# Deci-AI/super-gradients

Measured on NVIDIA H100. Metric: images/sec YOLO-NAS-S 640 bf16 train, higher is better.
Workload: dtype bf16

## Files before the change

include/sgb200.h:

```cpp
#ifndef SGB200_H_
#define SGB200_H_

#include <stdint.h>

#ifdef __cplusplus
extern "C" {
#endif

#define SGB_OK 0
#define SGB_E_INVALID (-1)
#define SGB_E_UNSUPPORTED (-2)
#define SGB_E_CUDA (-3)
#define SGB_E_ARCH (-4)

#define SGB_ACT_NONE 0
#define SGB_ACT_RELU 1
#define SGB_ACT_SILU 2

typedef uint16_t sgb_bf16;

typedef struct SgbConvDesc {
  int32_t N, H, W, C;
  int32_t K, R, S;
  int32_t P, Q;
// ... 10 lines not shown
  const sgb_bf16* residual;
  double* stats;
  int32_t stats_repl;
  int32_t act;
  int32_t out_f32;
} SgbEpilogue;

const char* sgb_last_error(void);
int sgb_version(void);
int sgb_check_device(void);
int64_t sgb_sm100_launches(void);
int64_t sgb_conv_halo_launches(void);
void sgb_conv_force_im2col(int on);
int64_t sgb_conv_wgrad_halo_launches(void);
void sgb_conv_wgrad_force_im2col(int on);

int sgb_conv_fprop(const SgbConvDesc* d, const sgb_bf16* x, const sgb_bf16* w_krsc, void* y, const SgbEpilogue* ep,
                   void* stream);
int sgb_conv_dgrad(const SgbConvDesc* d, const sgb_bf16* dy, const sgb_bf16* w_crsk, sgb_bf16* dx, int accumulate,
                   void* stream);
int sgb_conv_wgrad(const SgbConvDesc* d, const sgb_bf16* x, const sgb_bf16* dy, float* dw_krsc, void* stream);
int sgb_weight_prepare(const float* w_oihw, int K, int C, int R, int S, int c_pad, sgb_bf16* w_krsc, sgb_bf16* w_crsk,
                       const float* scale, int add_identity, void* stream);
int sgb_wgrad_to_oihw(const float* dw_krsc, int K, int C, int R, int S, int c_pad, float* g_oihw, int accumulate,
                      void* stream);
typedef struct SgbWeightItem {
  const float* w;
  const float* scale;
  sgb_bf16* krsc;
  sgb_bf16* crsk;
// ... 402 lines not shown
```

super_gradients_b200/csrc/capi.cu:

```cuda
#include <cstdarg>
#include <cstdio>

#include "common.cuh"
#include "conv_sm100.h"
#include "sm100_host.h"

static thread_local char g_err[512] = "";

void sgb_set_error(const char* fmt, ...) {
  va_list ap;
  va_start(ap, fmt);
  vsnprintf(g_err, sizeof(g_err), fmt, ap);
  va_end(ap);
}

int sgb_cuda_check(cudaError_t e, const char* what) {
  if (e == cudaSuccess) return SGB_OK;
  sgb_set_error("%s: %s", what, cudaGetErrorString(e));
  return SGB_E_CUDA;
}

extern "C" const char* sgb_last_error(void) { return g_err; }
extern "C" int sgb_version(void) { return 100; }
extern "C" int sgb_check_device(void) {
// ... 1 lines not shown
  if (int rc = sgb_cuda_check(cudaGetDevice(&dev), "cudaGetDevice")) return rc;
  cudaDeviceProp prop;
  if (int rc = sgb_cuda_check(cudaGetDeviceProperties(&prop, dev), "cudaGetDeviceProperties")) return rc;
  if (prop.major != 9) {
    sgb_set_error("libsgb200 is built for sm_90a only; device is sm_%d%d", prop.major, prop.minor);
    return SGB_E_ARCH;
  }
  return SGB_OK;
}

extern "C" int64_t sgb_sm100_launches(void) { return (int64_t)sm100::launch_count(); }
extern "C" int64_t sgb_conv_halo_launches(void) { return (int64_t)sm100::halo_launch_count(); }
extern "C" void sgb_conv_force_im2col(int on) { sm100::force_im2col(on != 0); }
extern "C" int64_t sgb_conv_wgrad_halo_launches(void) { return (int64_t)sm100::wgrad_halo_launch_count(); }
extern "C" void sgb_conv_wgrad_force_im2col(int on) { sm100::wgrad_force_im2col(on != 0); }
```

super_gradients_b200/csrc/conv_mma.cu:

```cuda
#include "common.cuh"
#include "conv_sm100.h"

namespace {

constexpr int BM = 128;
constexpr int BK = 32;
constexpr int STAGES = 4;
constexpr int THREADS = 256;

struct GatherClass {
  int M;
  int Hc, Wc;
  int nr, ns;
  int Kg;
  int hb_add, wb_add;
  int r0, s0;
  int oh_add, ow_add;
};

struct IGemmParams {
  const bf16* A;
  const bf16* B;
  void* Y;
  GatherClass cls[4];
// ... 574 lines not shown
  SGB_REQUIRE(s == 1 || s == 2, "dgrad supports stride 1 or 2");
  const int Kp = ((d->K + 7) / 8) * 8;
  if (s == 1 && d->pad == d->R / 2 && d->K % 16 == 0) {
    sm100::Problem q{};
    q.a = dy + d->y_off; q.N = d->N; q.H = d->P; q.W = d->Q; q.C = d->K; q.a_pitch = d->y_pitch;
    q.b = w_crsk; q.b_rows = d->C; q.b_cols = d->R * d->S * Kp; q.b_cols_per_tap = Kp;
    q.R = d->R; q.S = d->S; q.stride = 1; q.pad = d->R - 1 - d->pad; q.P = d->H; q.Q = d->W; q.flip = 1;
    q.y = dx; q.y_pitch = d->x_pitch; q.y_off = d->x_off;
    q.residual = accumulate ? dx : nullptr;
    q.stats_repl = 1;
    q.centre_from = d->centre_from;
    if (sm100::supported(q)) return sm100::launch(q, (cudaStream_t)stream);
  }
  if (s == 2 && d->K % 16 == 0 && d->R == 3 && d->S == 3 && d->pad == 1 && d->C % 8 == 0 && d->H % 2 == 0 &&
      d->W % 2 == 0 && d->H == 2 * d->P && d->W == 2 * d->Q) {
    bool all_ok = true;
    for (int cls = 0; cls < 4 && all_ok; ++cls) {
      const int ph = cls >> 1, pw = cls & 1;
      sm100::Problem q{};
      q.a = dy + d->y_off; q.N = d->N; q.H = d->P; q.W = d->Q; q.C = d->K; q.a_pitch = d->y_pitch;
      q.b = w_crsk; q.b_rows = d->C; q.b_cols = d->R * d->S * Kp; q.b_cols_per_tap = Kp;
      q.R = d->R; q.S = d->S; q.stride = 1; q.pad = 0; q.P = d->P; q.Q = d->Q; q.flip = 0;
      q.y = dx; q.y_pitch = d->x_pitch; q.y_off = d->x_off;
      q.residual = accumulate ? dx : nullptr;
      q.stats_repl = 1;
      q.out_mode = 1; q.o_mul = 2; q.oh_add = ph; q.ow_add = pw; q.outH = d->H; q.outW = d->W;
      int nt = 0;
      for (int r = 0; r < d->R; ++r) {
        if (((ph + d->pad - r) & 1) != 0) continue;
        for (int sx = 0; sx < d->S; ++sx) {
// ... 135 lines not shown
```

super_gradients_b200/csrc/conv_sm100.cu:

```cuda
#include <cuda.h>

#include <cstdlib>
#include <cstring>

#include "common.cuh"
#include "conv_sm100.h"
#include "sm100_host.h"
#include "sm100_ptx.cuh"

namespace sm100 {

constexpr int BLOCK_M = 128;
constexpr int NUM_THREADS = 384;
constexpr int CONSUMER_THREADS = 256;
constexpr int MAX_STAGES = 8;

struct Params {
  int M;
  int N;
  int C;
  int KC;
  int n_tiles;
  int stages;
  int P, Q;
// ... 244 lines not shown
        row_ok[h] = m < p.M;
        orow[h] = out_row(p, row_ok[h] ? m : 0);
      }
      tile_epilogue<BN>(p, acc, orow, row_ok, nt, wg, wq, lane, s_part, s_stats);
    }
  }
  __syncthreads();
  flush_stats(p, s_stats);
}

constexpr int HALO_W = 10, HALO_H = 10, HALO_TILE = 8;
constexpr uint32_t HALO_CG_BYTES = 1664;
constexpr uint32_t HALO_CTRL_BYTES = CTRL_BAR_BYTES + 16;
constexpr int HALO_MAX_STAGES = 6;

template <int BN, bool SKIP>
__global__ void __launch_bounds__(NUM_THREADS, BN <= 48 ? 2 : 1)
conv3x3_halo_kernel(const __grid_constant__ CUtensorMap map_a, const __grid_constant__ CUtensorMap map_b, const Params p) {
  extern __shared__ __align__(1024) unsigned char smem_raw[];
  const uint32_t smem_base = (smem_u32(smem_raw) + 1023u) & ~1023u;
  const int ksteps = p.C / 16;
  constexpr uint32_t b_box = BN * 32;
  const uint32_t b_bytes = 9u * ksteps * b_box;
  const uint32_t a_stage = ((uint32_t)(p.C / 8) * HALO_CG_BYTES + 1023u) & ~1023u;
  const uint32_t sb = smem_base, sa0 = smem_base + ((b_bytes + 1023u) & ~1023u);
  const uint32_t ctrl = sa0 + p.stages * a_stage;
  auto full_bar = [&](int s) { return ctrl + 8u * s; };
  auto empty_bar = [&](int s) { return ctrl + 8u * (MAX_STAGES + s); };
  const uint32_t b_bar = ctrl + CTRL_BAR_BYTES;
  float* s_part = reinterpret_cast<float*>(smem_raw + (ctrl + HALO_CTRL_BYTES - smem_u32(smem_raw)));
  float* s_stats = s_part + 8 * 2 * BN;

  const int warp = threadIdx.x >> 5, lane = threadIdx.x & 31;
  const int m_tiles = p.M;
  const int nt = blockIdx.x % p.n_tiles;
  const int mt_step = gridDim.x / p.n_tiles;
  const int mt0 = blockIdx.x / p.n_tiles;
  const int off = SKIP ? off_centre_steps<BN>(p, nt, ksteps, 16) : ksteps;

// ... 4 lines not shown
    }
    mbar_init(b_bar, 1);
    asm volatile("fence.mbarrier_init.release.cluster;" ::: "memory");
    asm volatile("fence.proxy.async.shared::cta;" ::: "memory");
  }
  if (p.stats)
    for (int i = threadIdx.x; i < 4 * p.N; i += NUM_THREADS) s_stats[i] = 0.f;
  __syncthreads();

  if (warp == 0) {
    if (elect_one()) {
      mbar_expect_tx(b_bar, (uint32_t)(8 * off + ksteps) * b_box);
      for (int bt = 0; bt < 9; ++bt)
        for (int ks = 0; ks < (bt == CENTRE_TAP ? ksteps : off); ++ks)
          tma_load_2d(sb + (uint32_t)(bt * ksteps + ks) * b_box, &map_b, b_bar, bt * p.b_cols_per_tap + 16 * ks, nt * BN);
      const uint32_t a_tx = (uint32_t)(p.C / 8) * (HALO_H * HALO_W * 16);
      int stg = 0;
      uint32_t par = 1;
      for (int mt = mt0; mt < m_tiles; mt += mt_step) {
        const int n_img = mt / p.halo_thw;
        const int rem = mt - n_img * p.halo_thw;
        const int th = rem / p.halo_tw, tw = rem - th * p.halo_tw;
        mbar_wait(empty_bar(stg), par);
        const uint32_t sa = sa0 + stg * a_stage;
        mbar_expect_tx(full_bar(stg), a_tx);
        for (int cg = 0; cg < p.C / 8; ++cg)
          tma_load_tiled_4d(sa + (uint32_t)cg * HALO_CG_BYTES, &map_a, full_bar(stg), 8 * cg, tw * HALO_TILE - 1, th * HALO_TILE - 1,
                            n_img);
        if (++stg == p.stages) {
          stg = 0;
          par ^= 1;
        }
      }
    }
  } else if (warp >= 4) {
    const int wg = (warp >> 2) - 1;
    const int wq = warp & 3;
    float acc[BN / 2];
    mbar_wait(b_bar, 0);
    for (int j = wg, mt = mt0 + wg * mt_step; mt < m_tiles; j += 2, mt += 2 * mt_step) {
      const int stg = j % p.stages;
      mbar_wait(full_bar(stg), (uint32_t)(j / p.stages) & 1u);
      const uint32_t sa = sa0 + stg * a_stage;
      wgmma_fence();
      int t = off > 0 ? 0 : CENTRE_TAP;
      uint32_t sa_t = sa + (uint32_t)((t / 3) * HALO_W + t % 3) * 16u, sb_t = sb + (uint32_t)(p.tap_b[t] * ksteps) * b_box;
      for (int k = 0, ks = 0, nk = 8 * off + ksteps; k < nk; ++k) {
        const uint64_t da = smem_desc_noswizzle(sa_t + (uint32_t)(2 * ks) * HALO_CG_BYTES, HALO_CG_BYTES, HALO_W * 16);
        const uint64_t db = smem_desc(sb_t + (uint32_t)ks * b_box, 32, 16u, 256u);
        mma_kk<BN>(acc, da, db, k != 0);
        if (++ks == (t == CENTRE_TAP ? ksteps : off) && ++t < 9) {
          ks = 0;
          sa_t = sa + (uint32_t)((t / 3) * HALO_W + t % 3) * 16u;
          sb_t = sb + (uint32_t)(p.tap_b[t] * ksteps) * b_box;
        }
      }
      wgmma_commit();
      wgmma_wait<0>();
      fence_regs(acc);
      __syncwarp();
      if (lane == 0) mbar_arrive(empty_bar(stg));

      const int n_img = mt / p.halo_thw;
      const int rem = mt - n_img * p.halo_thw;
      const int th = rem / p.halo_tw, tw = rem - th * p.halo_tw;
      const int ow = tw * HALO_TILE + (lane >> 2);
      long long orow[2];
      bool row_ok[2];
#pragma unroll
      for (int h = 0; h < 2; ++h) {
        const int oh = th * HALO_TILE + 2 * wq + h;
        row_ok[h] = oh < p.P && ow < p.Q;
        orow[h] = row_ok[h] ? ((long long)n_img * p.P + oh) * p.Q + ow : 0;
      }
      tile_epilogue<BN, 4>(p, acc, orow, row_ok, nt, wg, wq, lane, s_part + wg * 4 * 2 * BN, s_stats + wg * 2 * p.N);
    }
  }
  __syncthreads();
  if (p.stats) {
    for (int i = threadIdx.x; i < 2 * p.N; i += NUM_THREADS) s_stats[i] += s_stats[2 * p.N + i];
    __syncthreads();
  }
  flush_stats(p, s_stats);
}

struct WParams {
  int K, C;
  int R, S, stride, pad, P, Q;
  int npix;
  int CB;
// ... 124 lines not shown
        }
      }
    }
  }
}

constexpr uint32_t WH_A_BYTES = WPIX * 128;

__host__ __device__ constexpr uint32_t wgrad_halo_stage_bytes(int nb) {
  return (WH_A_BYTES + (uint32_t)(nb / 8) * HALO_CG_BYTES + 1023u) & ~1023u;
}

template <int NB, int NT>
__device__ __forceinline__ void wgrad_halo_consume(const WParams& p, uint32_t ring, uint32_t bars, int t0, int t1, int tap0, int rb,
                                                   int ctile) {
  constexpr uint32_t stage_bytes = wgrad_halo_stage_bytes(NB);
  const int wq = (threadIdx.x >> 5) & 3, lane = threadIdx.x & 31;
  auto full_bar = [&](int s) { return bars + 8u * s; };
  auto empty_bar = [&](int s) { return bars + 8u * (MAX_STAGES + s); };
  float acc[NT > 0 ? NT : 1][NB / 2];
  int stg = 0, prev = 0;
  uint32_t par = 0;
  for (int mt = t0; mt < t1; ++mt) {
    mbar_wait(full_bar(stg), par);
    if constexpr (NT > 0) {
      const uint32_t sa = ring + stg * stage_bytes, sx = sa + WH_A_BYTES;
      wgmma_fence();
#pragma unroll
      for (int t = 0; t < NT; ++t) {
        const int tap = tap0 + t;
        const uint32_t sx_t = sx + (uint32_t)((tap / 3) * HALO_W + tap % 3) * 16u;
#pragma unroll
        for (int j = 0; j < WPIX / 16; ++j) {
          const uint64_t da = smem_desc(sa + (uint32_t)j * 16u * 128u, 128, WPIX * 128, 8 * 128);
          const uint64_t db = smem_desc_noswizzle(sx_t + (uint32_t)j * 2u * HALO_W * 16u, HALO_W * 16, HALO_CG_BYTES);
          mma_mn<NB>(acc[t], da, db, (mt != t0 || j != 0) ? 1u : 0u);
        }
      }
      wgmma_commit();
      wgmma_wait<1>();
    }
    __syncwarp();
    if (lane == 0 && mt != t0) mbar_arrive(empty_bar(prev));
    prev = stg;
    if (++stg == p.stages) {
      stg = 0;
      par ^= 1;
    }
  }
  if constexpr (NT > 0) {
// ... 15 lines not shown
#pragma unroll
          for (int j = 0; j < NB / 8; ++j)
            asm volatile("red.global.add.v2.f32 [%0], {%1, %2};" ::"l"(drow + t * p.cpad + 8 * j), "f"(acc[t][4 * j + 2 * h]),
                         "f"(acc[t][4 * j + 2 * h + 1])
                         : "memory");
      }
    }
  }
}

template <int NB>
__global__ void __launch_bounds__(NUM_THREADS, 1)
wgrad3x3_halo_kernel(const __grid_constant__ CUtensorMap map_dy, const __grid_constant__ CUtensorMap map_x, const WParams p) {
  extern __shared__ __align__(1024) unsigned char smem_raw[];
  const uint32_t smem_base = (smem_u32(smem_raw) + 1023u) & ~1023u;
  constexpr uint32_t a_bytes = WH_A_BYTES, stage_bytes = wgrad_halo_stage_bytes(NB);
  const uint32_t ctrl = smem_base + p.stages * stage_bytes;
  auto full_bar = [&](int s) { return ctrl + 8u * s; };
  auto empty_bar = [&](int s) { return ctrl + 8u * (MAX_STAGES + s); };

  const int warp = threadIdx.x >> 5;
  const int items = p.rb_all * p.n_ctiles;
  const int split = blockIdx.x / items, item = blockIdx.x - split * items;
  const int ctile = item / p.rb_all, rb = item - ctile * p.rb_all;
  const bool all_taps = rb < p.rb_off;
  const int t0 = split * p.tiles_per_cta, t1 = min(t0 + p.tiles_per_cta, p.tiles);

  if (threadIdx.x == 0) {
    for (int s = 0; s < p.stages; ++s) {
      mbar_init(full_bar(s), 1);
      mbar_init(empty_bar(s), 8);
    }
    asm volatile("fence.mbarrier_init.release.cluster;" ::: "memory");
    asm volatile("fence.proxy.async.shared::cta;" ::: "memory");
  }
  __syncthreads();

  if (warp == 0) {
    if (elect_one()) {
      const uint32_t tx = a_bytes + (NB / 8) * (HALO_H * HALO_W * 16);
      int stg = 0;
      uint32_t par = 1;
      for (int mt = t0; mt < t1; ++mt) {
        const int n_img = mt / p.halo_thw;
        const int rem = mt - n_img * p.halo_thw;
        const int th = rem / p.halo_tw, tw = rem - th * p.halo_tw;
        mbar_wait(empty_bar(stg), par);
        const uint32_t sa = smem_base + stg * stage_bytes;
        mbar_expect_tx(full_bar(stg), tx);
        tma_load_tiled_4d(sa, &map_dy, full_bar(stg), 64 * rb, tw * HALO_TILE, th * HALO_TILE, n_img);
        for (int cg = 0; cg < NB / 8; ++cg)
          tma_load_tiled_4d(sa + a_bytes + (uint32_t)cg * HALO_CG_BYTES, &map_x, full_bar(stg), ctile * NB + 8 * cg,
                            tw * HALO_TILE - 1, th * HALO_TILE - 1, n_img);
        if (++stg == p.stages) {
          stg = 0;
          par ^= 1;
        }
      }
    }
  } else if (warp >= 4) {
    const int wg = (warp >> 2) - 1;
    const uint32_t ring = smem_base, bars = ctrl;
    if (!all_taps && wg == 0)
      wgrad_halo_consume<NB, 1>(p, ring, bars, t0, t1, CENTRE_TAP, rb, ctile);
    else if (!all_taps)
      wgrad_halo_consume<NB, 0>(p, ring, bars, t0, t1, 0, rb, ctile);
    else if (wg == 0)
      wgrad_halo_consume<NB, 5>(p, ring, bars, t0, t1, 0, rb, ctile);
    else
      wgrad_halo_consume<NB, 4>(p, ring, bars, t0, t1, 5, rb, ctile);
  }
}

EncodeTiledFn g_tiled = nullptr;
EncodeIm2colFn g_im2col = nullptr;
int g_num_sms = 0;
long long g_launches = 0;
long long g_halo_launches = 0;
long long g_wgrad_halo_launches = 0;
bool g_force_im2col = false;
bool g_wgrad_force_im2col = false;
long long launch_count() { return g_launches; }
long long halo_launch_count() { return g_halo_launches; }
long long wgrad_halo_launch_count() { return g_wgrad_halo_launches; }
void force_im2col(bool on) { g_force_im2col = on; }
void wgrad_force_im2col(bool on) { g_wgrad_force_im2col = on; }

int init_driver() {
  if (g_tiled && g_im2col) return SGB_OK;
  cudaDriverEntryPointQueryResult qres;
  void* fn = nullptr;
  if (cudaGetDriverEntryPoint("cuTensorMapEncodeTiled", &fn, cudaEnableDefault, &qres) != cudaSuccess || !fn) {
    sgb_set_error("cuTensorMapEncodeTiled entry point not found");
    return SGB_E_CUDA;
  }
  g_tiled = (EncodeTiledFn)fn;
  fn = nullptr;
  if (cudaGetDriverEntryPoint("cuTensorMapEncodeIm2col", &fn, cudaEnableDefault, &qres) != cudaSuccess || !fn) {
    sgb_set_error("cuTensorMapEncodeIm2col entry point not found");
    return SGB_E_CUDA;
  }
// ... 33 lines not shown
Variant<ConvFn> g_conv[] = {{16, conv_wgmma_kernel<16, false>, 0, false},   {32, conv_wgmma_kernel<32, false>, 0, false},
                            {48, conv_wgmma_kernel<48, false>, 0, false},   {64, conv_wgmma_kernel<64, false>, 0, false},
                            {96, conv_wgmma_kernel<96, false>, 0, false},   {128, conv_wgmma_kernel<128, false>, 0, false}};
Variant<ConvFn> g_conv_skip[] = {{16, conv_wgmma_kernel<16, true>, 0, false},   {32, conv_wgmma_kernel<32, true>, 0, false},
                                 {48, conv_wgmma_kernel<48, true>, 0, false},   {64, conv_wgmma_kernel<64, true>, 0, false},
                                 {96, conv_wgmma_kernel<96, true>, 0, false},   {128, conv_wgmma_kernel<128, true>, 0, false}};
Variant<ConvFn> g_halo[] = {{16, conv3x3_halo_kernel<16, false>, 0, false},   {32, conv3x3_halo_kernel<32, false>, 0, false},
                            {48, conv3x3_halo_kernel<48, false>, 0, false},   {64, conv3x3_halo_kernel<64, false>, 0, false},
                            {96, conv3x3_halo_kernel<96, false>, 0, false},   {128, conv3x3_halo_kernel<128, false>, 0, false}};
Variant<ConvFn> g_halo_skip[] = {{16, conv3x3_halo_kernel<16, true>, 0, false},   {32, conv3x3_halo_kernel<32, true>, 0, false},
                                 {48, conv3x3_halo_kernel<48, true>, 0, false},   {64, conv3x3_halo_kernel<64, true>, 0, false},
                                 {96, conv3x3_halo_kernel<96, true>, 0, false},   {128, conv3x3_halo_kernel<128, true>, 0, false}};
Variant<WgradFn> g_wgrad[] = {{16, wgrad_wgmma_kernel<16>, 0, false}, {32, wgrad_wgmma_kernel<32>, 0, false},
                              {48, wgrad_wgmma_kernel<48>, 0, false}, {64, wgrad_wgmma_kernel<64>, 0, false},
                              {96, wgrad_wgmma_kernel<96>, 0, false}, {128, wgrad_wgmma_kernel<128>, 0, false}};
Variant<WgradFn> g_wgrad_halo[] = {{16, wgrad3x3_halo_kernel<16>, 0, false}, {32, wgrad3x3_halo_kernel<32>, 0, false},
                                   {48, wgrad3x3_halo_kernel<48>, 0, false}};

template <class Fn>
int prepare(Variant<Fn>& v, const char* what) {
  if (v.ready) return SGB_OK;
  if (int rc = sgb_cuda_check(cudaFuncSetAttribute(v.fn, cudaFuncAttributeMaxDynamicSharedMemorySize, 227 * 1024), what)) return rc;
  cudaFuncAttributes fa{};
  if (int rc = sgb_cuda_check(cudaFuncGetAttributes(&fa, v.fn), what)) return rc;
  v.regs = fa.numRegs;
  v.ready = true;
  return SGB_OK;
}

int pick_bn(int n) {
  for (int bn : {16, 32, 48, 64, 96, 128})
    if (n <= bn) return bn;
  int best = 128, best_waste = (n + 127) / 128 * 128 - n;
  for (int bn : {96, 64}) {
    const int waste = (n + bn - 1) / bn * bn - n;
    if (waste < best_waste) { best_waste = waste; best = bn; }
  }
  return best;
}

size_t halo_smem(int C, int bn, int n, bool stats, int stages) {
  const size_t b_bytes = ((size_t)9 * C * bn * 2 + 1023) & ~(size_t)1023;
  const size_t a_stage = ((size_t)(C / 8) * HALO_CG_BYTES + 1023) & ~(size_t)1023;
  return 1024 + b_bytes + (size_t)stages * a_stage + HALO_CTRL_BYTES + (stats ? (size_t)(8 * 2 * bn + 4 * n) * 4 : 0);
}

bool halo_tiles_fit(int P, int Q) {
  const long long covered = (long long)((P + 7) / 8) * 8 * ((Q + 7) / 8) * 8;
  return 20ll * P * Q >= 17 * covered;
}

int halo_bn(const Problem& q) {
  if (q.R != 3 || q.S != 3 || q.stride != 1 || q.pad != 1 || q.ntaps > 0 || q.out_mode != 0) return 0;
  if (q.P != q.H || q.Q != q.W) return 0;
  if (!halo_tiles_fit(q.P, q.Q)) return 0;
  const int n = q.b_rows, full = pick_bn(n);
  auto waste = [&](int bn) { return (n + bn - 1) / bn * bn - n; };
  for (int bn : {full, 96, 64})
    if (bn <= full && (bn == full || (q.C <= 96 && bn >= 64 && waste(bn) <= waste(full))) &&
        halo_smem(q.C, bn, n, q.stats != nullptr, 2) <= 227 * 1024)
      return bn;
  return 0;
}

int encode_halo_map(CUtensorMap* map, const void* x, int N, int H, int W, int C, int pitch) {
  cuuint64_t dims[4] = {(cuuint64_t)C, (cuuint64_t)W, (cuuint64_t)H, (cuuint64_t)N};
  cuuint64_t strides[3] = {(cuuint64_t)pitch * 2, (cuuint64_t)W * pitch * 2, (cuuint64_t)H * W * pitch * 2};
  cuuint32_t box[4] = {8, HALO_W, HALO_H, 1};
  cuuint32_t estr[4] = {1, 1, 1, 1};
  CUresult r = g_tiled(map, CU_TENSOR_MAP_DATA_TYPE_BFLOAT16, 4, const_cast<void*>(x), dims, strides, box, estr, CU_TENSOR_MAP_INTERLEAVE_NONE,
                       CU_TENSOR_MAP_SWIZZLE_NONE, CU_TENSOR_MAP_L2_PROMOTION_L2_128B, CU_TENSOR_MAP_FLOAT_OOB_FILL_NONE);
  if (r != CUDA_SUCCESS) {
    sgb_set_error("cuTensorMapEncodeTiled(halo) failed with %d (C=%d W=%d H=%d N=%d pitch=%d)", (int)r, C, W, H, N, pitch);
    return SGB_E_CUDA;
  }
  return SGB_OK;
}

int launch_halo(const Problem& q, const Params& p0, int bn, cudaStream_t st) {
  Params p = p0;
  p.n_tiles = (p.N + bn - 1) / bn;
  p.halo_tw = (q.Q + HALO_TILE - 1) / HALO_TILE;
  p.halo_thw = p.halo_tw * ((q.P + HALO_TILE - 1) / HALO_TILE);
  p.M = q.N * p.halo_thw;
  p.centre_n = 0;
  Variant<ConvFn>* var = nullptr;
  for (auto& v : p.centre_c > 0 ? g_halo_skip : g_halo)
    if (v.bn == bn) var = &v;
  if (int rc = prepare(*var, "conv3x3_halo_kernel")) return rc;
  const int regs_alloc = ((var->regs + 7) / 8) * 8 * NUM_THREADS;
  int ctas_per_sm = 65536 / regs_alloc;
  if (ctas_per_sm > 2) ctas_per_sm = 2;
  if (ctas_per_sm < 1) ctas_per_sm = 1;
  int stages = 0;
  for (;; --ctas_per_sm) {
    const size_t budget = (ctas_per_sm == 1 ? 227u : 227u / ctas_per_sm - 1u) * 1024u;
    for (stages = HALO_MAX_STAGES; stages >= 2 && halo_smem(q.C, bn, p.N, p.stats != nullptr, stages) > budget; --stages) {
    }
    if (stages >= 2 || ctas_per_sm == 1) break;
  }
  if (stages < 2) { sgb_set_error("conv3x3_halo: tile does not fit shared memory"); return SGB_E_UNSUPPORTED; }
  p.stages = stages;
  const size_t smem = halo_smem(q.C, bn, p.N, p.stats != nullptr, stages);

  alignas(64) CUtensorMap map_a, map_b;
  if (int rc = encode_halo_map(&map_a, q.a, q.N, q.H, q.W, q.C, q.a_pitch)) return rc;
  {
    cuuint64_t dims[2] = {(cuuint64_t)q.b_cols, (cuuint64_t)q.b_rows};
    cuuint64_t strides[1] = {(cuuint64_t)q.b_cols * 2};
    cuuint32_t box[2] = {16, (cuuint32_t)bn};
    cuuint32_t estr[2] = {1, 1};
    CUresult r = g_tiled(&map_b, CU_TENSOR_MAP_DATA_TYPE_BFLOAT16, 2, const_cast<void*>(q.b), dims, strides, box, estr,
                         CU_TENSOR_MAP_INTERLEAVE_NONE, CU_TENSOR_MAP_SWIZZLE_32B, CU_TENSOR_MAP_L2_PROMOTION_L2_128B,
                         CU_TENSOR_MAP_FLOAT_OOB_FILL_NONE);
    if (r != CUDA_SUCCESS) {
      sgb_set_error("cuTensorMapEncodeTiled(halo B) failed with %d (cols=%d rows=%d BN=%d)", (int)r, q.b_cols, q.b_rows, bn);
      return SGB_E_CUDA;
    }
  }
  int per_nt = g_num_sms * ctas_per_sm / p.n_tiles;
  if (per_nt > p.M) per_nt = p.M;
  if (per_nt < 1) per_nt = 1;
  var->fn<<<per_nt * p.n_tiles, NUM_THREADS, smem, st>>>(map_a, map_b, p);
  ++g_launches;
  ++g_halo_launches;
  return sgb_cuda_check(cudaGetLastError(), "conv3x3_halo_kernel");
}

}

int launch(const Problem& q, cudaStream_t st) {
  if (int rc = init_driver()) return rc;
  Params p{};
  p.M = q.N * q.P * q.Q;
  p.N = q.b_rows;
  p.C = q.C;
  p.KC = q.C % 64 == 0 ? 64 : (q.C % 32 == 0 ? 32 : 16);
  if (p.KC < 64 && q.C > 32) p.KC = 64;
  const int bn = pick_bn(p.N);
  p.n_tiles = (p.N + bn - 1) / bn;
// ... 8 lines not shown
      p.tap_dw[t] = (signed char)(t % q.S);
      p.tap_b[t] = (signed char)(q.flip ? (p.ntaps - 1 - t) : t);
    }
  }
  if (p.ntaps > 9) return SGB_E_UNSUPPORTED;
  p.out_mode = q.out_mode; p.o_mul = q.o_mul; p.oh_add = q.oh_add; p.ow_add = q.ow_add; p.outH = q.outH; p.outW = q.outW;
  p.b_cols_per_tap = q.b_cols_per_tap;
  p.y = (bf16*)q.y; p.y_pitch = q.y_pitch; p.y_off = q.y_off;
  p.scale = q.scale; p.shift = q.shift; p.residual = (const bf16*)q.residual;
  p.stats = q.stats; p.stats_repl = q.stats_repl > 0 ? q.stats_repl : 1; p.act = q.act;
  if (q.centre_from > 0) {
    if (q.R != 3 || q.S != 3 || q.stride != 1 || q.pad != 1 || q.ntaps > 0 || q.centre_from % 16 != 0 ||
        q.centre_from >= (q.flip ? q.C : q.b_rows))
      return SGB_E_INVALID;
    (q.flip ? p.centre_c : p.centre_n) = q.centre_from;
  }
  if (!g_force_im2col)
    if (const int hbn = halo_bn(q)) return launch_halo(q, p, hbn, st);
  Variant<ConvFn>* var = nullptr;
  for (auto& v : p.centre_n > 0 || p.centre_c > 0 ? g_conv_skip : g_conv)
    if (v.bn == bn) var = &v;
  if (int rc = prepare(*var, "conv_wgmma_kernel")) return rc;
  const uint32_t a_bytes = BLOCK_M * p.KC * 2, b_bytes = ((uint32_t)(bn * p.KC * 2) + 1023u) & ~1023u;
  const uint32_t stage_bytes = a_bytes + b_bytes;
  const uint32_t ctrl_bytes = CTRL_BAR_BYTES + (p.stats ? (uint32_t)(8 * 2 * bn + 2 * p.N) * 4u : 0u);
  const int regs_alloc = ((var->regs + 7) / 8) * 8 * NUM_THREADS;
  int ctas_per_sm = 65536 / regs_alloc;
  if (ctas_per_sm > 2) ctas_per_sm = 2;
  if (ctas_per_sm < 1) ctas_per_sm = 1;
  int stages = 0;
// ... 91 lines not shown

  alignas(64) CUtensorMap map_dy, map_x;
  {
    cuuint64_t dims[4] = {(cuuint64_t)q.K, (cuuint64_t)q.Q, (cuuint64_t)q.P, (cuuint64_t)q.N};
    cuuint64_t strides[3] = {(cuuint64_t)q.y_pitch * 2, (cuuint64_t)q.Q * q.y_pitch * 2, (cuuint64_t)q.P * q.Q * q.y_pitch * 2};
    cuuint32_t box[4] = {64, HALO_TILE, HALO_TILE, 1};
    cuuint32_t estr[4] = {1, 1, 1, 1};
    CUresult r = g_tiled(&map_dy, CU_TENSOR_MAP_DATA_TYPE_BFLOAT16, 4, const_cast<void*>(q.dy), dims, strides, box, estr,
                         CU_TENSOR_MAP_INTERLEAVE_NONE, CU_TENSOR_MAP_SWIZZLE_128B, CU_TENSOR_MAP_L2_PROMOTION_L2_128B,
                         CU_TENSOR_MAP_FLOAT_OOB_FILL_NONE);
    if (r != CUDA_SUCCESS) {
      sgb_set_error("cuTensorMapEncodeTiled(dy tile) failed with %d (K=%d Q=%d P=%d N=%d pitch=%d)", (int)r, q.K, q.Q, q.P, q.N, q.y_pitch);
      return SGB_E_CUDA;
    }
  }
  if (int rc = encode_halo_map(&map_x, q.x, q.N, q.H, q.W, q.C, q.x_pitch)) return rc;
  var->fn<<<splits * items, NUM_THREADS, smem, st>>>(map_dy, map_x, p);
  ++g_launches;
  ++g_wgrad_halo_launches;
  return sgb_cuda_check(cudaGetLastError(), "wgrad3x3_halo_kernel");
}

}

int wgrad_launch(const WgradProblem& q, cudaStream_t st) {
  if (int rc = init_driver()) return rc;
  WParams p{};
  p.K = q.K; p.C = q.C; p.R = q.R; p.S = q.S; p.stride = q.stride; p.pad = q.pad; p.P = q.P; p.Q = q.Q;
  p.npix = q.N * q.P * q.Q;
  int nb = 16;
  for (int cand : {128, 96, 64, 48, 32})
// ... 65 lines not shown
```

super_gradients_b200/csrc/conv_sm100.h:

```cpp
#pragma once
#include <cuda_runtime.h>

namespace sm100 {

struct Problem {
  const void* a;
  int N, H, W, C, a_pitch;
  const void* b;
  int b_rows, b_cols, b_cols_per_tap;
  int R, S, stride, pad, P, Q, flip;
  int ntaps;
  int tap_dh[9], tap_dw[9], tap_b[9];
  int out_mode, o_mul, oh_add, ow_add, outH, outW;
  void* y;
  int y_pitch, y_off;
  const float* scale;
  const float* shift;
  const void* residual;
  double* stats;
  int stats_repl, act;
  int centre_from;
};

struct WgradProblem {
  const void* x;
  const void* dy;
  int N, H, W, C, x_pitch;
  int K, y_pitch;
  int R, S, stride, pad, P, Q;
  float* dw;
  int centre_from;
};

bool wgrad_supported(const WgradProblem& q);
int wgrad_launch(const WgradProblem& q, cudaStream_t st);
bool supported(const Problem& q);
int launch(const Problem& q, cudaStream_t st);
long long launch_count();
long long halo_launch_count();
void force_im2col(bool on);
long long wgrad_halo_launch_count();
void wgrad_force_im2col(bool on);

}
```

super_gradients_b200/lib.py:

```python
import ctypes
import os
from ctypes import POINTER, Structure, c_char_p, c_double, c_float, c_int, c_int32, c_int64, c_void_p

_HERE = os.path.dirname(os.path.abspath(__file__))
LIB_PATH = os.path.join(_HERE, "libsgb200.so")

ACT_NONE, ACT_RELU, ACT_SILU = 0, 1, 2


class SgbError(RuntimeError):
    pass


class ConvDesc(Structure):
    _fields_ = [(n, c_int32) for n in ("N", "H", "W", "C", "K", "R", "S", "P", "Q", "stride", "pad", "x_pitch", "x_off", "y_pitch", "y_off", "up2", "centre_from")]


class Epilogue(Structure):
    _fields_ = [
        ("scale", c_void_p),
        ("shift", c_void_p),
        ("residual", c_void_p),
        ("stats", c_void_p),
        ("stats_repl", c_int32),
# ... 121 lines not shown
    ]


P = c_void_p
_I, _F, _L = c_int, c_float, c_int64

_SIGNATURES = {
    "sgb_last_error": (c_char_p, []),
    "sgb_version": (c_int, []),
    "sgb_check_device": (c_int, []),
    "sgb_sm100_launches": (c_int64, []),
    "sgb_conv_halo_launches": (c_int64, []),
    "sgb_conv_force_im2col": (None, [_I]),
    "sgb_conv_wgrad_halo_launches": (c_int64, []),
    "sgb_conv_wgrad_force_im2col": (None, [_I]),
    "sgb_conv_fprop": (c_int, [POINTER(ConvDesc), P, P, P, POINTER(Epilogue), P]),
    "sgb_conv_dgrad": (c_int, [POINTER(ConvDesc), P, P, P, _I, P]),
    "sgb_conv_wgrad": (c_int, [POINTER(ConvDesc), P, P, P, P]),
    "sgb_weight_prepare": (c_int, [P, _I, _I, _I, _I, _I, P, P, P, _I, P]),
    "sgb_wgrad_to_oihw": (c_int, [P, _I, _I, _I, _I, _I, P, _I, P]),
    "sgb_weight_prepare_batch": (c_int, [P, _I, c_int64, P]),
    "sgb_wgrad_to_oihw_batch": (c_int, [P, _I, c_int64, P]),
    "sgb_qarep_alpha_finish_batch": (c_int, [P, _I, P]),
    "sgb_convt2x2_fprop": (c_int, [POINTER(ConvDesc), P, P, P, P, P]),
    "sgb_nchw_f32_to_nhwc_bf16": (c_int, [P, _I, _I, _I, _I, P, _I, _I, _I, P]),
    "sgb_stem_patches_f32": (c_int, [P, _I, _I, _I, _I, _I, _I, _I, P, _I, _I, _I, P]),
    "sgb_nhwc_bf16_to_nchw_f32": (c_int, [P, _I, _I, _I, _I, _I, _I, P, P]),
    "sgb_bn_act_fwd": (c_int, [POINTER(BnDesc), P, P, P, P, P, P, P, P, P, P, P]),
    "sgb_bn_act_fwd_fused": (c_int, [POINTER(BnDesc), P, P, P, P, P, P, P, P, P, P, P]),
    "sgb_bn_act_infer": (c_int, [POINTER(BnDesc), P, P, P, P, P, P, P, P]),
# ... 48 lines not shown
    "sgb_sgd_step": (c_int, [P, P, P, _L, P, P]),
    "sgb_adamw_step": (c_int, [P, P, P, P, _L, P, P]),
    "sgb_ema_update": (c_int, [P, P, _L, P, P]),
    "sgb_adam_step": (c_int, [P, P, P, P, _L, P, P]),
    "sgb_rmsprop_step": (c_int, [P, P, P, P, P, _L, P, P]),
    "sgb_rmsprop_tf_step": (c_int, [P, P, P, P, P, _L, P, P]),
    "sgb_lion_step": (c_int, [P, P, P, _L, P, P]),
    "sgb_lamb_grad_sqnorm": (c_int, [P, P, c_int32, P, P, P]),
    "sgb_lamb_step": (c_int, [P, P, P, P, P, _L, P, c_int32, P, P, P]),
    "sgb_clip_grad_norm": (c_int, [P, P, c_int32, P, c_int32, c_int32, _F, P, P, P]),
    "sgb_average_snapshots": (c_int, [P, c_int32, _L, P, P]),
}

_lib = None

LAUNCH_COUNT = {"sgb_tal_assign": 4, "sgb_lamb_step": 2, "sgb_clip_grad_norm": 2, "sgb_atss_assign": 3, "sgb_pose_tal_assign": 4, "sgb_sm100_launches": 0, "sgb_conv_halo_launches": 0, "sgb_conv_force_im2col": 0, "sgb_conv_wgrad_halo_launches": 0, "sgb_conv_wgrad_force_im2col": 0, "sgb_sliding_window_merge_workspace_bytes": 0, "sgb_sliding_window_merge_launches": 0, "sgb_last_error": 0, "sgb_version": 0, "sgb_check_device": 0}
LAUNCHES = [0]


def exported_names():
    return sorted(_SIGNATURES)


def load():
    global _lib
    if _lib is not None:
        return _lib
    if not os.path.exists(LIB_PATH):
        raise SgbError(f"{LIB_PATH} not found: run `python -c 'import __graft_entry__ as g; g.build()'` " "(there is no non-CUDA fallback for this package)")
    lib = ctypes.CDLL(LIB_PATH)
    for name, (res, args) in _SIGNATURES.items():
# ... 21 lines not shown
```

Baseline: 959.7.

## Add halo-tiled TMA kernels for stride-2 3x3 conv fprop and dgrad

Generalizes the 3x3 halo conv kernel with a Halo<KIND> policy so it handles stride-2 forward convolutions (four strided TMA planes) and stride-2 dgrad. The dgrad variant computes all four output parity classes in one launch from a single shared halo tile, instead of four separate per-tap launches. The aim is to cut launches and repeated dy loads, and to avoid im2col for stride-2 layers. The cost is more template variants, lower occupancy for the dgrad kernel (launch bounds forced to 1), and a per-tap fallback behind a debug switch.

Result: no change. 968.1 (median of 6 runs) (+0.9%).

```diff
diff --git a/include/sgb200.h b/include/sgb200.h
--- a/include/sgb200.h
+++ b/include/sgb200.h
@@ -48,6 +48,8 @@
 void sgb_conv_force_im2col(int on);
 int64_t sgb_conv_wgrad_halo_launches(void);
 void sgb_conv_wgrad_force_im2col(int on);
+int64_t sgb_conv_halo_s2_launches(void);
+void sgb_conv_halo_s2_force_per_tap(int on);
 
 int sgb_conv_fprop(const SgbConvDesc* d, const sgb_bf16* x, const sgb_bf16* w_krsc, void* y, const SgbEpilogue* ep,
                    void* stream);
diff --git a/super_gradients_b200/csrc/capi.cu b/super_gradients_b200/csrc/capi.cu
--- a/super_gradients_b200/csrc/capi.cu
+++ b/super_gradients_b200/csrc/capi.cu
@@ -39,3 +39,5 @@
 extern "C" void sgb_conv_force_im2col(int on) { sm100::force_im2col(on != 0); }
 extern "C" int64_t sgb_conv_wgrad_halo_launches(void) { return (int64_t)sm100::wgrad_halo_launch_count(); }
 extern "C" void sgb_conv_wgrad_force_im2col(int on) { sm100::wgrad_force_im2col(on != 0); }
+extern "C" int64_t sgb_conv_halo_s2_launches(void) { return (int64_t)sm100::s2_halo_launch_count(); }
+extern "C" void sgb_conv_halo_s2_force_per_tap(int on) { sm100::s2_force_per_tap(on != 0); }
diff --git a/super_gradients_b200/csrc/conv_mma.cu b/super_gradients_b200/csrc/conv_mma.cu
--- a/super_gradients_b200/csrc/conv_mma.cu
+++ b/super_gradients_b200/csrc/conv_mma.cu
@@ -612,6 +612,32 @@
   }
   if (s == 2 && d->K % 16 == 0 && d->R == 3 && d->S == 3 && d->pad == 1 && d->C % 8 == 0 && d->H % 2 == 0 &&
       d->W % 2 == 0 && d->H == 2 * d->P && d->W == 2 * d->Q) {
+    {
+      sm100::Problem q{};
+      q.a = dy + d->y_off; q.N = d->N; q.H = d->P; q.W = d->Q; q.C = d->K; q.a_pitch = d->y_pitch;
+      q.b = w_crsk; q.b_rows = d->C; q.b_cols = d->R * d->S * Kp; q.b_cols_per_tap = Kp;
+      q.R = d->R; q.S = d->S; q.stride = 1; q.pad = 0; q.P = d->P; q.Q = d->Q; q.flip = 0;
+      q.y = dx; q.y_pitch = d->x_pitch; q.y_off = d->x_off;
+      q.residual = accumulate ? dx : nullptr;
+      q.stats_repl = 1;
+      q.out_mode = 1; q.o_mul = 2; q.outH = d->H; q.outW = d->W;
+      q.s2_dgrad = 1;
+      for (int cls = 0; cls < 4; ++cls) {
+        const int ph = cls >> 1, pw = cls & 1;
+        for (int r = 0; r < 3; ++r)
+          for (int sx = 0; sx < 3; ++sx)
+            if (((ph + 1 - r) & 1) == 0 && ((pw + 1 - sx) & 1) == 0) {
+              q.tap_dh[q.ntaps] = (ph + 1 - r) / 2;
+              q.tap_dw[q.ntaps] = (pw + 1 - sx) / 2;
+              q.tap_b[q.ntaps] = r * 3 + sx;
+              ++q.ntaps;
+            }
+      }
+      if (sm100::supported(q)) {
+        const int rc = sm100::launch(q, (cudaStream_t)stream);
+        if (rc != SGB_E_UNSUPPORTED) return rc;
+      }
+    }
     bool all_ok = true;
     for (int cls = 0; cls < 4 && all_ok; ++cls) {
       const int ph = cls >> 1, pw = cls & 1;
diff --git a/super_gradients_b200/csrc/conv_sm100.cu b/super_gradients_b200/csrc/conv_sm100.cu
--- a/super_gradients_b200/csrc/conv_sm100.cu
+++ b/super_gradients_b200/csrc/conv_sm100.cu
@@ -282,15 +282,42 @@
 constexpr uint32_t HALO_CTRL_BYTES = CTRL_BAR_BYTES + 16;
 constexpr int HALO_MAX_STAGES = 6;
 
-template <int BN, bool SKIP>
-__global__ void __launch_bounds__(NUM_THREADS, BN <= 48 ? 2 : 1)
+constexpr int S2_PLANE_W = 9;
+constexpr uint32_t S2_CG_BYTES = 1408;
+
+
+enum HaloKind { HALO_S1 = 1, HALO_S2 = 2, HALO_S2_DGRAD = 3 };
+template <int KIND>
+struct Halo {
+  static constexpr int W = KIND == HALO_S1 ? HALO_W : S2_PLANE_W;
+  static constexpr int PLANES = KIND == HALO_S2 ? 4 : 1;
+  static constexpr uint32_t CG = KIND == HALO_S1 ? HALO_CG_BYTES : S2_CG_BYTES;
+  static constexpr uint32_t TX = W * W * 16;
+  static __device__ __forceinline__ uint32_t tap_offset(int dh, int dw, int groups) {
+    if (KIND != HALO_S2) return (uint32_t)(dh * W + dw) * 16u;
+    return (uint32_t)(((dh & 1) * 2 + (dw & 1)) * groups) * S2_CG_BYTES + (uint32_t)((dh >> 1) * S2_PLANE_W + (dw >> 1)) * 16u;
+  }
+  static __device__ __forceinline__ void load(uint32_t dst, const CUtensorMap* map, uint32_t bar, int c0, int groups, int h0, int w0,
+                                              int n) {
+    constexpr int step = KIND == HALO_S2 ? 2 : 1, origin = KIND == HALO_S2_DGRAD ? 0 : -1;
+    for (int pl = 0; pl < PLANES; ++pl)
+      for (int cg = 0; cg < groups; ++cg)
+        tma_load_tiled_4d(dst + (uint32_t)(pl * groups + cg) * CG, map, bar, c0 + 8 * cg, step * w0 + origin + (pl & 1),
+                          step * h0 + origin + (pl >> 1), n);
+  }
+};
+
+template <int BN, bool SKIP, int KIND = HALO_S1>
+__global__ void __launch_bounds__(NUM_THREADS, BN <= 48 && KIND != HALO_S2_DGRAD ? 2 : 1)
 conv3x3_halo_kernel(const __grid_constant__ CUtensorMap map_a, const __grid_constant__ CUtensorMap map_b, const Params p) {
   extern __shared__ __align__(1024) unsigned char smem_raw[];
   const uint32_t smem_base = (smem_u32(smem_raw) + 1023u) & ~1023u;
   const int ksteps = p.C / 16;
   constexpr uint32_t b_box = BN * 32;
   const uint32_t b_bytes = 9u * ksteps * b_box;
-  const uint32_t a_stage = ((uint32_t)(p.C / 8) * HALO_CG_BYTES + 1023u) & ~1023u;
+  using G = Halo<KIND>;
+  const int groups = p.C / 8;
+  const uint32_t a_stage = ((uint32_t)(G::PLANES * groups) * G::CG + 1023u) & ~1023u;
   const uint32_t sb = smem_base, sa0 = smem_base + ((b_bytes + 1023u) & ~1023u);
   const uint32_t ctrl = sa0 + p.stages * a_stage;
   auto full_bar = [&](int s) { return ctrl + 8u * s; };
@@ -325,7 +352,7 @@
       for (int bt = 0; bt < 9; ++bt)
         for (int ks = 0; ks < (bt == CENTRE_TAP ? ksteps : off); ++ks)
           tma_load_2d(sb + (uint32_t)(bt * ksteps + ks) * b_box, &map_b, b_bar, bt * p.b_cols_per_tap + 16 * ks, nt * BN);
-      const uint32_t a_tx = (uint32_t)(p.C / 8) * (HALO_H * HALO_W * 16);
+      const uint32_t a_tx = (uint32_t)(G::PLANES * groups) * G::TX;
       int stg = 0;
       uint32_t par = 1;
       for (int mt = mt0; mt < m_tiles; mt += mt_step) {
@@ -335,9 +362,7 @@
         mbar_wait(empty_bar(stg), par);
         const uint32_t sa = sa0 + stg * a_stage;
         mbar_expect_tx(full_bar(stg), a_tx);
-        for (int cg = 0; cg < p.C / 8; ++cg)
-          tma_load_tiled_4d(sa + (uint32_t)cg * HALO_CG_BYTES, &map_a, full_bar(stg), 8 * cg, tw * HALO_TILE - 1, th * HALO_TILE - 1,
-                            n_img);
+        G::load(sa, &map_a, full_bar(stg), 0, groups, th * HALO_TILE, tw * HALO_TILE, n_img);
         if (++stg == p.stages) {
           stg = 0;
           par ^= 1;
@@ -353,38 +378,75 @@
       const int stg = j % p.stages;
       mbar_wait(full_bar(stg), (uint32_t)(j / p.stages) & 1u);
       const uint32_t sa = sa0 + stg * a_stage;
-      wgmma_fence();
-      int t = off > 0 ? 0 : CENTRE_TAP;
-      uint32_t sa_t = sa + (uint32_t)((t / 3) * HALO_W + t % 3) * 16u, sb_t = sb + (uint32_t)(p.tap_b[t] * ksteps) * b_box;
-      for (int k = 0, ks = 0, nk = 8 * off + ksteps; k < nk; ++k) {
-        const uint64_t da = smem_desc_noswizzle(sa_t + (uint32_t)(2 * ks) * HALO_CG_BYTES, HALO_CG_BYTES, HALO_W * 16);
-        const uint64_t db = smem_desc(sb_t + (uint32_t)ks * b_box, 32, 16u, 256u);
-        mma_kk<BN>(acc, da, db, k != 0);
-        if (++ks == (t == CENTRE_TAP ? ksteps : off) && ++t < 9) {
-          ks = 0;
-          sa_t = sa + (uint32_t)((t / 3) * HALO_W + t % 3) * 16u;
-          sb_t = sb + (uint32_t)(p.tap_b[t] * ksteps) * b_box;
-        }
-      }
-      wgmma_commit();
-      wgmma_wait<0>();
-      fence_regs(acc);
-      __syncwarp();
-      if (lane == 0) mbar_arrive(empty_bar(stg));
-
-      const int n_img = mt / p.halo_thw;
-      const int rem = mt - n_img * p.halo_thw;
-      const int th = rem / p.halo_tw, tw = rem - th * p.halo_tw;
-      const int ow = tw * HALO_TILE + (lane >> 2);
-      long long orow[2];
-      bool row_ok[2];
-#pragma unroll
-      for (int h = 0; h < 2; ++h) {
-        const int oh = th * HALO_TILE + 2 * wq + h;
-        row_ok[h] = oh < p.P && ow < p.Q;
-        orow[h] = row_ok[h] ? ((long long)n_img * p.P + oh) * p.Q + ow : 0;
-      }
-      tile_epilogue<BN, 4>(p, acc, orow, row_ok, nt, wg, wq, lane, s_part + wg * 4 * 2 * BN, s_stats + wg * 2 * p.N);
+      if constexpr (KIND == HALO_S2_DGRAD) {
+        const int n_img = mt / p.halo_thw;
+        const int rem = mt - n_img * p.halo_thw;
+        const int th = rem / p.halo_tw, tw = rem - th * p.halo_tw;
+        const int i = tw * HALO_TILE + (lane >> 2);
+        for (int c = 0; c < 4; ++c) {
+          const int first = c == 0 ? 0 : 2 * c - 1, last = first + (c == 0 ? 1 : (c == 3 ? 4 : 2));
+          int t = first;
+          uint32_t sa_t = sa + G::tap_offset(p.tap_dh[t], p.tap_dw[t], groups), sb_t = sb + (uint32_t)(p.tap_b[t] * ksteps) * b_box;
+          wgmma_fence();
+          for (int k = 0, ks = 0, nk = (last - first) * ksteps; k < nk; ++k) {
+            const uint64_t da = smem_desc_noswizzle(sa_t + (uint32_t)(2 * ks) * G::CG, G::CG, G::W * 16);
+            const uint64_t db = smem_desc(sb_t + (uint32_t)ks * b_box, 32, 16u, 256u);
+            mma_kk<BN>(acc, da, db, k != 0);
+            if (++ks == ksteps && ++t < last) {
+              ks = 0;
+              sa_t = sa + G::tap_offset(p.tap_dh[t], p.tap_dw[t], groups);
+              sb_t = sb + (uint32_t)(p.tap_b[t] * ksteps) * b_box;
+            }
+          }
+          wgmma_commit();
+          wgmma_wait<0>();
+          fence_regs(acc);
+          __syncwarp();
+          if (c == 3 && lane == 0) mbar_arrive(empty_bar(stg));
+          long long orow[2];
+          bool row_ok[2];
+#pragma unroll
+          for (int h = 0; h < 2; ++h) {
+            const int j = th * HALO_TILE + 2 * wq + h;
+            row_ok[h] = j < p.P && i < p.Q;
+            orow[h] = row_ok[h] ? ((long long)n_img * p.outH + 2 * j + (c >> 1)) * p.outW + 2 * i + (c & 1) : 0;
+          }
+          tile_epilogue<BN, 4>(p, acc, orow, row_ok, nt, wg, wq, lane, s_part + wg * 4 * 2 * BN, s_stats + wg * 2 * p.N);
+        }
+      } else {
+        wgmma_fence();
+        int t = off > 0 ? 0 : CENTRE_TAP;
+        uint32_t sa_t = sa + G::tap_offset(t / 3, t % 3, groups), sb_t = sb + (uint32_t)(p.tap_b[t] * ksteps) * b_box;
+        for (int k = 0, ks = 0, nk = 8 * off + ksteps; k < nk; ++k) {
+          const uint64_t da = smem_desc_noswizzle(sa_t + (uint32_t)(2 * ks) * G::CG, G::CG, G::W * 16);
+          const uint64_t db = smem_desc(sb_t + (uint32_t)ks * b_box, 32, 16u, 256u);
+          mma_kk<BN>(acc, da, db, k != 0);
+          if (++ks == (t == CENTRE_TAP ? ksteps : off) && ++t < 9) {
+            ks = 0;
+            sa_t = sa + G::tap_offset(t / 3, t % 3, groups);
+            sb_t = sb + (uint32_t)(p.tap_b[t] * ksteps) * b_box;
+          }
+        }
+        wgmma_commit();
+        wgmma_wait<0>();
+        fence_regs(acc);
+        __syncwarp();
+        if (lane == 0) mbar_arrive(empty_bar(stg));
+
+        const int n_img = mt / p.halo_thw;
+        const int rem = mt - n_img * p.halo_thw;
+        const int th = rem / p.halo_tw, tw = rem - th * p.halo_tw;
+        const int ow = tw * HALO_TILE + (lane >> 2);
+        long long orow[2];
+        bool row_ok[2];
+#pragma unroll
+        for (int h = 0; h < 2; ++h) {
+          const int oh = th * HALO_TILE + 2 * wq + h;
+          row_ok[h] = oh < p.P && ow < p.Q;
+          orow[h] = row_ok[h] ? ((long long)n_img * p.P + oh) * p.Q + ow : 0;
+        }
+        tile_epilogue<BN, 4>(p, acc, orow, row_ok, nt, wg, wq, lane, s_part + wg * 4 * 2 * BN, s_stats + wg * 2 * p.N);
+      }
     }
   }
   __syncthreads();
@@ -539,6 +601,7 @@
 template <int NB, int NT>
 __device__ __forceinline__ void wgrad_halo_consume(const WParams& p, uint32_t ring, uint32_t bars, int t0, int t1, int tap0, int rb,
                                                    int ctile) {
+  using G = Halo<1>;
   constexpr uint32_t stage_bytes = wgrad_halo_stage_bytes(NB);
   const int wq = (threadIdx.x >> 5) & 3, lane = threadIdx.x & 31;
   auto full_bar = [&](int s) { return bars + 8u * s; };
@@ -554,11 +617,11 @@
 #pragma unroll
       for (int t = 0; t < NT; ++t) {
         const int tap = tap0 + t;
-        const uint32_t sx_t = sx + (uint32_t)((tap / 3) * HALO_W + tap % 3) * 16u;
+        const uint32_t sx_t = sx + G::tap_offset(tap / 3, tap % 3, NB / 8);
 #pragma unroll
         for (int j = 0; j < WPIX / 16; ++j) {
           const uint64_t da = smem_desc(sa + (uint32_t)j * 16u * 128u, 128, WPIX * 128, 8 * 128);
-          const uint64_t db = smem_desc_noswizzle(sx_t + (uint32_t)j * 2u * HALO_W * 16u, HALO_W * 16, HALO_CG_BYTES);
+          const uint64_t db = smem_desc_noswizzle(sx_t + (uint32_t)j * 2u * G::W * 16u, G::W * 16, G::CG);
           mma_mn<NB>(acc[t], da, db, (mt != t0 || j != 0) ? 1u : 0u);
         }
       }
@@ -604,6 +667,7 @@
 wgrad3x3_halo_kernel(const __grid_constant__ CUtensorMap map_dy, const __grid_constant__ CUtensorMap map_x, const WParams p) {
   extern __shared__ __align__(1024) unsigned char smem_raw[];
   const uint32_t smem_base = (smem_u32(smem_raw) + 1023u) & ~1023u;
+  using G = Halo<1>;
   constexpr uint32_t a_bytes = WH_A_BYTES, stage_bytes = wgrad_halo_stage_bytes(NB);
   const uint32_t ctrl = smem_base + p.stages * stage_bytes;
   auto full_bar = [&](int s) { return ctrl + 8u * s; };
@@ -628,7 +692,7 @@
 
   if (warp == 0) {
     if (elect_one()) {
-      const uint32_t tx = a_bytes + (NB / 8) * (HALO_H * HALO_W * 16);
+      const uint32_t tx = a_bytes + (uint32_t)(G::PLANES * (NB / 8)) * G::TX;
       int stg = 0;
       uint32_t par = 1;
       for (int mt = t0; mt < t1; ++mt) {
@@ -639,9 +703,7 @@
         const uint32_t sa = smem_base + stg * stage_bytes;
         mbar_expect_tx(full_bar(stg), tx);
         tma_load_tiled_4d(sa, &map_dy, full_bar(stg), 64 * rb, tw * HALO_TILE, th * HALO_TILE, n_img);
-        for (int cg = 0; cg < NB / 8; ++cg)
-          tma_load_tiled_4d(sa + a_bytes + (uint32_t)cg * HALO_CG_BYTES, &map_x, full_bar(stg), ctile * NB + 8 * cg,
-                            tw * HALO_TILE - 1, th * HALO_TILE - 1, n_img);
+        G::load(sa + a_bytes, &map_x, full_bar(stg), ctile * NB, NB / 8, th * HALO_TILE, tw * HALO_TILE, n_img);
         if (++stg == p.stages) {
           stg = 0;
           par ^= 1;
@@ -668,13 +730,17 @@
 long long g_launches = 0;
 long long g_halo_launches = 0;
 long long g_wgrad_halo_launches = 0;
+long long g_s2_halo_launches = 0;
 bool g_force_im2col = false;
 bool g_wgrad_force_im2col = false;
+bool g_s2_force_per_tap = false;
 long long launch_count() { return g_launches; }
 long long halo_launch_count() { return g_halo_launches; }
 long long wgrad_halo_launch_count() { return g_wgrad_halo_launches; }
+long long s2_halo_launch_count() { return g_s2_halo_launches; }
 void force_im2col(bool on) { g_force_im2col = on; }
 void wgrad_force_im2col(bool on) { g_wgrad_force_im2col = on; }
+void s2_force_per_tap(bool on) { g_s2_force_per_tap = on; }
 
 int init_driver() {
   if (g_tiled && g_im2col) return SGB_OK;
@@ -738,6 +804,13 @@
 Variant<WgradFn> g_wgrad[] = {{16, wgrad_wgmma_kernel<16>, 0, false}, {32, wgrad_wgmma_kernel<32>, 0, false},
                               {48, wgrad_wgmma_kernel<48>, 0, false}, {64, wgrad_wgmma_kernel<64>, 0, false},
                               {96, wgrad_wgmma_kernel<96>, 0, false}, {128, wgrad_wgmma_kernel<128>, 0, false}};
+Variant<ConvFn> g_halo_s2[] = {{16, conv3x3_halo_kernel<16, false, HALO_S2>, 0, false},   {32, conv3x3_halo_kernel<32, false, HALO_S2>, 0, false},
+                               {48, conv3x3_halo_kernel<48, false, HALO_S2>, 0, false},   {64, conv3x3_halo_kernel<64, false, HALO_S2>, 0, false},
+                               {96, conv3x3_halo_kernel<96, false, HALO_S2>, 0, false},   {128, conv3x3_halo_kernel<128, false, HALO_S2>, 0, false}};
+Variant<ConvFn> g_halo_s2_dgrad[] = {
+    {16, conv3x3_halo_kernel<16, false, HALO_S2_DGRAD>, 0, false}, {32, conv3x3_halo_kernel<32, false, HALO_S2_DGRAD>, 0, false},
+    {48, conv3x3_halo_kernel<48, false, HALO_S2_DGRAD>, 0, false}, {64, conv3x3_halo_kernel<64, false, HALO_S2_DGRAD>, 0, false},
+    {96, conv3x3_halo_kernel<96, false, HALO_S2_DGRAD>, 0, false}, {128, conv3x3_halo_kernel<128, false, HALO_S2_DGRAD>, 0, false}};
 Variant<WgradFn> g_wgrad_halo[] = {{16, wgrad3x3_halo_kernel<16>, 0, false}, {32, wgrad3x3_halo_kernel<32>, 0, false},
                                    {48, wgrad3x3_halo_kernel<48>, 0, false}};
 
@@ -763,9 +836,11 @@
   return best;
 }
 
-size_t halo_smem(int C, int bn, int n, bool stats, int stages) {
+int halo_kind(const Problem& q) { return q.s2_dgrad ? HALO_S2_DGRAD : (q.stride == 2 ? HALO_S2 : HALO_S1); }
+size_t halo_smem(int C, int bn, int n, bool stats, int stages, int kind) {
   const size_t b_bytes = ((size_t)9 * C * bn * 2 + 1023) & ~(size_t)1023;
-  const size_t a_stage = ((size_t)(C / 8) * HALO_CG_BYTES + 1023) & ~(size_t)1023;
+  const size_t cg_bytes = kind == HALO_S1 ? HALO_CG_BYTES : (kind == HALO_S2 ? 4 * S2_CG_BYTES : S2_CG_BYTES);
+  const size_t a_stage = ((size_t)(C / 8) * cg_bytes + 1023) & ~(size_t)1023;
   return 1024 + b_bytes + (size_t)stages * a_stage + HALO_CTRL_BYTES + (stats ? (size_t)(8 * 2 * bn + 4 * n) * 4 : 0);
 }
 
@@ -775,23 +850,28 @@
 }
 
 int halo_bn(const Problem& q) {
-  if (q.R != 3 || q.S != 3 || q.stride != 1 || q.pad != 1 || q.ntaps > 0 || q.out_mode != 0) return 0;
-  if (q.P != q.H || q.Q != q.W) return 0;
+  if (q.s2_dgrad) {
+    if (g_s2_force_per_tap) return 0;
+  } else {
+    if (q.R != 3 || q.S != 3 || q.pad != 1 || q.ntaps > 0 || q.out_mode != 0) return 0;
+    if (q.stride == 1 ? (q.P != q.H || q.Q != q.W) : (g_s2_force_per_tap || q.H != 2 * q.P || q.W != 2 * q.Q || q.C > 48)) return 0;
+  }
   if (!halo_tiles_fit(q.P, q.Q)) return 0;
   const int n = q.b_rows, full = pick_bn(n);
   auto waste = [&](int bn) { return (n + bn - 1) / bn * bn - n; };
   for (int bn : {full, 96, 64})
     if (bn <= full && (bn == full || (q.C <= 96 && bn >= 64 && waste(bn) <= waste(full))) &&
-        halo_smem(q.C, bn, n, q.stats != nullptr, 2) <= 227 * 1024)
+        halo_smem(q.C, bn, n, q.stats != nullptr, 2, halo_kind(q)) <= 227 * 1024)
       return bn;
   return 0;
 }
 
-int encode_halo_map(CUtensorMap* map, const void* x, int N, int H, int W, int C, int pitch) {
+int encode_halo_map(CUtensorMap* map, const void* x, int N, int H, int W, int C, int pitch, int kind) {
   cuuint64_t dims[4] = {(cuuint64_t)C, (cuuint64_t)W, (cuuint64_t)H, (cuuint64_t)N};
   cuuint64_t strides[3] = {(cuuint64_t)pitch * 2, (cuuint64_t)W * pitch * 2, (cuuint64_t)H * W * pitch * 2};
-  cuuint32_t box[4] = {8, HALO_W, HALO_H, 1};
-  cuuint32_t estr[4] = {1, 1, 1, 1};
+  const cuuint32_t step = kind == HALO_S2 ? 2 : 1, side = kind == HALO_S1 ? HALO_W : step * S2_PLANE_W;
+  cuuint32_t box[4] = {8, side, side, 1};
+  cuuint32_t estr[4] = {1, step, step, 1};
   CUresult r = g_tiled(map, CU_TENSOR_MAP_DATA_TYPE_BFLOAT16, 4, const_cast<void*>(x), dims, strides, box, estr, CU_TENSOR_MAP_INTERLEAVE_NONE,
                        CU_TENSOR_MAP_SWIZZLE_NONE, CU_TENSOR_MAP_L2_PROMOTION_L2_128B, CU_TENSOR_MAP_FLOAT_OOB_FILL_NONE);
   if (r != CUDA_SUCCESS) {
@@ -809,7 +889,8 @@
   p.M = q.N * p.halo_thw;
   p.centre_n = 0;
   Variant<ConvFn>* var = nullptr;
-  for (auto& v : p.centre_c > 0 ? g_halo_skip : g_halo)
+  const int kind = halo_kind(q);
+  for (auto& v : kind == HALO_S2_DGRAD ? g_halo_s2_dgrad : kind == HALO_S2 ? g_halo_s2 : (p.centre_c > 0 ? g_halo_skip : g_halo))
     if (v.bn == bn) var = &v;
   if (int rc = prepare(*var, "conv3x3_halo_kernel")) return rc;
   const int regs_alloc = ((var->regs + 7) / 8) * 8 * NUM_THREADS;
@@ -819,16 +900,16 @@
   int stages = 0;
   for (;; --ctas_per_sm) {
     const size_t budget = (ctas_per_sm == 1 ? 227u : 227u / ctas_per_sm - 1u) * 1024u;
-    for (stages = HALO_MAX_STAGES; stages >= 2 && halo_smem(q.C, bn, p.N, p.stats != nullptr, stages) > budget; --stages) {
+    for (stages = HALO_MAX_STAGES; stages >= 2 && halo_smem(q.C, bn, p.N, p.stats != nullptr, stages, kind) > budget; --stages) {
     }
     if (stages >= 2 || ctas_per_sm == 1) break;
   }
   if (stages < 2) { sgb_set_error("conv3x3_halo: tile does not fit shared memory"); return SGB_E_UNSUPPORTED; }
   p.stages = stages;
-  const size_t smem = halo_smem(q.C, bn, p.N, p.stats != nullptr, stages);
+  const size_t smem = halo_smem(q.C, bn, p.N, p.stats != nullptr, stages, kind);
 
   alignas(64) CUtensorMap map_a, map_b;
-  if (int rc = encode_halo_map(&map_a, q.a, q.N, q.H, q.W, q.C, q.a_pitch)) return rc;
+  if (int rc = encode_halo_map(&map_a, q.a, q.N, q.H, q.W, q.C, q.a_pitch, kind)) return rc;
   {
     cuuint64_t dims[2] = {(cuuint64_t)q.b_cols, (cuuint64_t)q.b_rows};
     cuuint64_t strides[1] = {(cuuint64_t)q.b_cols * 2};
@@ -847,7 +928,7 @@
   if (per_nt < 1) per_nt = 1;
   var->fn<<<per_nt * p.n_tiles, NUM_THREADS, smem, st>>>(map_a, map_b, p);
   ++g_launches;
-  ++g_halo_launches;
+  ++(kind == HALO_S1 ? g_halo_launches : g_s2_halo_launches);
   return sgb_cuda_check(cudaGetLastError(), "conv3x3_halo_kernel");
 }
 
@@ -886,6 +967,10 @@
         q.centre_from >= (q.flip ? q.C : q.b_rows))
       return SGB_E_INVALID;
     (q.flip ? p.centre_c : p.centre_n) = q.centre_from;
+  }
+  if (q.s2_dgrad) {
+    const int hbn = halo_bn(q);
+    return hbn ? launch_halo(q, p, hbn, st) : SGB_E_UNSUPPORTED;
   }
   if (!g_force_im2col)
     if (const int hbn = halo_bn(q)) return launch_halo(q, p, hbn, st);
@@ -1007,7 +1092,7 @@
       return SGB_E_CUDA;
     }
   }
-  if (int rc = encode_halo_map(&map_x, q.x, q.N, q.H, q.W, q.C, q.x_pitch)) return rc;
+  if (int rc = encode_halo_map(&map_x, q.x, q.N, q.H, q.W, q.C, q.x_pitch, HALO_S1)) return rc;
   var->fn<<<splits * items, NUM_THREADS, smem, st>>>(map_dy, map_x, p);
   ++g_launches;
   ++g_wgrad_halo_launches;
diff --git a/super_gradients_b200/csrc/conv_sm100.h b/super_gradients_b200/csrc/conv_sm100.h
--- a/super_gradients_b200/csrc/conv_sm100.h
+++ b/super_gradients_b200/csrc/conv_sm100.h
@@ -20,6 +20,7 @@
   double* stats;
   int stats_repl, act;
   int centre_from;
+  int s2_dgrad;
 };
 
 struct WgradProblem {
@@ -41,5 +42,7 @@
 void force_im2col(bool on);
 long long wgrad_halo_launch_count();
 void wgrad_force_im2col(bool on);
+long long s2_halo_launch_count();
+void s2_force_per_tap(bool on);
 
 }
diff --git a/super_gradients_b200/lib.py b/super_gradients_b200/lib.py
--- a/super_gradients_b200/lib.py
+++ b/super_gradients_b200/lib.py
@@ -159,6 +159,8 @@
     "sgb_conv_force_im2col": (None, [_I]),
     "sgb_conv_wgrad_halo_launches": (c_int64, []),
     "sgb_conv_wgrad_force_im2col": (None, [_I]),
+    "sgb_conv_halo_s2_launches": (c_int64, []),
+    "sgb_conv_halo_s2_force_per_tap": (None, [_I]),
     "sgb_conv_fprop": (c_int, [POINTER(ConvDesc), P, P, P, POINTER(Epilogue), P]),
     "sgb_conv_dgrad": (c_int, [POINTER(ConvDesc), P, P, P, _I, P]),
     "sgb_conv_wgrad": (c_int, [POINTER(ConvDesc), P, P, P, P]),
@@ -237,7 +239,7 @@
 
 _lib = None
 
-LAUNCH_COUNT = {"sgb_tal_assign": 4, "sgb_lamb_step": 2, "sgb_clip_grad_norm": 2, "sgb_atss_assign": 3, "sgb_pose_tal_assign": 4, "sgb_sm100_launches": 0, "sgb_conv_halo_launches": 0, "sgb_conv_force_im2col": 0, "sgb_conv_wgrad_halo_launches": 0, "sgb_conv_wgrad_force_im2col": 0, "sgb_sliding_window_merge_workspace_bytes": 0, "sgb_sliding_window_merge_launches": 0, "sgb_last_error": 0, "sgb_version": 0, "sgb_check_device": 0}
+LAUNCH_COUNT = {"sgb_tal_assign": 4, "sgb_lamb_step": 2, "sgb_clip_grad_norm": 2, "sgb_atss_assign": 3, "sgb_pose_tal_assign": 4, "sgb_sm100_launches": 0, "sgb_conv_halo_launches": 0, "sgb_conv_force_im2col": 0, "sgb_conv_wgrad_halo_launches": 0, "sgb_conv_wgrad_force_im2col": 0, "sgb_conv_halo_s2_launches": 0, "sgb_conv_halo_s2_force_per_tap": 0, "sgb_sliding_window_merge_workspace_bytes": 0, "sgb_sliding_window_merge_launches": 0, "sgb_last_error": 0, "sgb_version": 0, "sgb_check_device": 0}
 LAUNCHES = [0]
 
 
```
